# joe5saia/Hmc.jl

Hardware: AMD Instinct MI355X
Metric: Gibbs draws/sec (whole node), 3-state T=1000 x256 windows per GPU (higher is better)
Workload: dtype f64

## Files before the change

### hmc.jl_amd/csrc/gibbs_device.hpp

```cpp
#pragma once
#include <hip/hip_runtime.h>
#include <stdint.h>

#include "../../include/hmcg.h"
#include "round5.hpp"

namespace hmcg {

enum { SITE_SIG2 = 0, SITE_MU = 1, SITE_RHO = 2, SITE_A = 3, SITE_X = 4, SITE_NOISE = 5 };
constexpr int GAMMA_MAX_ATTEMPTS = 64;
constexpr double INVSQRT2PI = 0.3989422804014327;
constexpr double TWO_PI = 6.283185307179586476925286766559;
constexpr double EPS64 = 2.220446049250313e-16;

struct KernelParams {
    const double* Y;
    const int32_t* T;
    const double* yreal;
    int32_t ldY, W, H;
    int32_t sweep_begin;
    int32_t sweep_end;
    int32_t resume;
    int32_t final_launch;
    int32_t horizons[HMCG_MAXH];
    uint32_t seed_lo, seed_hi, window_base;
    double alpha, nu;
    double* mu; double* sig2; double* A; double* pi_end; double* fcast; double* summary;
    int32_t* status;
    const int32_t* x_init; int32_t* x_final; double* pif_final; uint8_t* xstate; double* sumacc;
    const uint32_t* window_ids;
    unsigned long long* dbg;
    int32_t per_sample, burnin_s, nrun_s, n_samples, nd;
    int32_t nd_ld, draw_off;
    double kappa;
    const int32_t* sig_range;
// ... 527 lines not shown

template <int K, int L, int NT, bool SIG>
struct SweepShared {
    static constexpr int NW = NT / 64;
    static constexpr int NCNT = K + K * K;
    static constexpr int NF = K * K + (SIG ? K : 0);
    static constexpr int FW = (64 * L < 1024) ? 10 : 16;
    static constexpr int FPK = 32 / FW;
    static constexpr int NPK = (NF + FPK - 1) / FPK;
    unsigned red_pk[NW][NPK];
    double red_s1[SIG ? NW : 1][K];
    double red_s2[SIG ? NW : 1][K];
    int x_end;
    double red_d1[NW][K];
    double red_d2[NW][K];
    double pivot[K];
    ThetaBuf<K> th[2];
    RngBuf<K> rb[2];
    double wtot[NW][K * K];
    double pfirst[NT + 1][K];
    uint32_t wmap[NW];
    double ulast;
    int xfirst[NT + 1];
    double bred[NW];
    int selcnt[2][8][3];
    double ux[NT * L];
    double exptab[EXPTAB_N * EXPTAB_C];
    struct OutConst { double* base; double yr; int packed; int h; };
    OutConst oc[2][64];
    double ftail[2][SIG ? HMCG_MAXTAIL : 1][K];
    double pf_rep[2][K];
    double y_last[2];
};

template <int NW>
__device__ __forceinline__ double block_sum(double v, double* bred, int wave, int lane)
{
    v = wave_sum(v);
    __syncthreads();
    if (lane == 0 && wave < NW) bred[wave] = v;
    __syncthreads();
    double t = 0.0;
#pragma unroll
    for (int w = 0; w < NW; ++w) t += bred[w];
    return t;
}
template <int NW>
__device__ __forceinline__ double block_minmax(double v, double* bred, int wave, int lane, bool is_max)
{
    v = is_max ? wave_max(v) : wave_min(v);
    __syncthreads();
    if (lane == 0 && wave < NW) bred[wave] = v;
    __syncthreads();
    double t = bred[0];
#pragma unroll
    for (int w = 1; w < NW; ++w) t = is_max ? fmax(t, bred[w]) : fmin(t, bred[w]);
    return t;
}

__device__ __forceinline__ unsigned long long order_key(double v)
{
    const long long b = __double_as_longlong(v + 0.0);
    return (unsigned long long)(b ^ ((b >> 63) | (long long)0x8000000000000000ull));
}
__device__ __forceinline__ double key_value(unsigned long long k)
{
// ... 31 lines not shown
        for (int w = 0; w < NW; ++w) { t0 += cnt[par][w][0]; t1 += cnt[par][w][1]; t2 += cnt[par][w][2]; }
        t0 = __builtin_amdgcn_readfirstlane(t0); t1 = __builtin_amdgcn_readfirstlane(t1); t2 = __builtin_amdgcn_readfirstlane(t2);
        unsigned long long digit = 0ull;
        if (r >= t0) { r -= t0; digit = 1ull;
            if (r >= t1) { r -= t1; digit = 2ull;
                if (r >= t2) { r -= t2; digit = 3ull; } } }
        prefix |= digit << b;
        mask |= 3ull << b;
    }
    return prefix;
}

template <int K>
__device__ __forceinline__ void sort_order(const double (&mu)[K], int (&order)[K])
{
    int pos[K];
#pragma unroll
    for (int i = 0; i < K; ++i) {
        int c = 0;
#pragma unroll
        for (int j = 0; j < K; ++j) c += (mu[j] < mu[i] || (mu[j] == mu[i] && j < i)) ? 1 : 0;
        pos[i] = c;
    }
#pragma unroll
    for (int q = 0; q < K; ++q) {
        int o = 0;
#pragma unroll
        for (int i = 0; i < K; ++i) o += (pos[i] == q) ? i : 0;
        order[q] = o;
    }
}

#ifdef HMCG_STAMPS
#define HMCG_NSTAMP 20
#define HMCG_NSTAMP_ALL (HMCG_NSTAMP + 2)
#define STAMP(i)                                                          \
    do {                                                                  \
        __builtin_amdgcn_sched_barrier(0);                                \
        asm volatile("; HMCG_STAMP_MARK %0" :: "n"(i));                    \
        const unsigned long long t_ = __builtin_amdgcn_s_memtime();       \
        __builtin_amdgcn_s_waitcnt(0xC07F);                               \
        __builtin_amdgcn_sched_barrier(0);                                \
        stamp_acc[i] += t_ - stamp_prev;                                  \
        stamp_prev = t_;                                                  \
    } while (0)
#else
#define STAMP(i)
#endif


template <int K, int L, int NT, bool SIG = false, bool SMOOTH = false, int NH = 0, int OCC = 1>
__global__ __launch_bounds__(NT + 64 * NH) __attribute__((amdgpu_waves_per_eu(OCC)))
void gibbs_sweeps_kernel(const KernelParams p)
{
    static_assert(NH == 0 || (NH == 4 && NT == 256), "helper waves: 256 + 256 threads");
    static_assert(K >= 2 && K <= 4, "small-K kernel: byte-per-entry state maps (v_perm_b32 composition)");
    static_assert(NT % 64 == 0 && NT >= 128, "at least two whole waves (wave 0 draws, the others work in its shadow)");
    constexpr int NW = NT / 64;
    constexpr int KK = K * K;
    constexpr int NG = K + KK;
    static_assert(NG <= 64, "draw roles must fit wave 0");
    using Sh = SweepShared<K, L, NT, SIG>;
    __shared__ Sh sh;

    int w_ = blockIdx.x;
    int t_lo_ = INT32_MIN, t_hi_ = INT32_MAX;
    if (p.order) {
        const int n_live = p.order[0];
        t_lo_ = p.order[1]; t_hi_ = p.order[2];
        if (n_live >= 0) {
            if (w_ >= n_live) __builtin_amdgcn_endpgm();
            w_ = p.order[4 + w_];
        }
    }
    const int w = w_;
    const int tid = threadIdx.x, lane = tid & 63, wave = __builtin_amdgcn_readfirstlane(tid >> 6);
    const int T = p.T[w];
    const int t0 = tid * L;
    const int owner = (T - 1) / L, l_last = (T - 1) % L;
    const bool helper = NH > 0 && __builtin_amdgcn_readfirstlane(wave) >= NW;
    int st = 0;

    if (T < t_lo_ || T > t_hi_) __builtin_amdgcn_endpgm();
    if (T < 2 || T > NT * L || T > p.ldY) {
        if (tid == 0) flag_skipped(p, w, HMCG_ST_BAD_T);
        return;
    }

    exptab_fill(sh.exptab, tid, NT + 64 * NH);
    constexpr int XPAD = K < 4 ? K : 0;
    constexpr bool PADMARK = K < 4;
    double y[L];
    int x[L];
    bool bad = false;
#pragma unroll
// ... 134 lines not shown
            const bool live = task < NTASK;
            const bool t_rho = task < K;
            const bool t_gx = !t_rho && task < K + 2 * NG;
            const bool t_z = !t_rho && !t_gx && task < 2 * K + 2 * NG;
            const bool t_gl = !t_rho && !t_gx && !t_z;
            const int gt = t_gx ? task - K : task - (2 * K + 2 * NG);
            const int role = gt >> 1, j = gt & 1;
            uint32_t site = SITE_RHO, elem = (uint32_t)task, idx = 0;
            if (t_gx || t_gl) {
                site = role < K ? SITE_SIG2 : SITE_A;
                elem = role < K ? (uint32_t)role : (uint32_t)(role - K);
                idx = 2u * (uint32_t)j + (t_gl ? 1u : 0u);
            } else if (t_z) {
                site = SITE_MU; elem = (uint32_t)(task - (K + 2 * NG));
            }
            uint32_t r[4];
            g.block(site, elem, idx, r);
            const double uraw = u53(r[0], r[1]);
            const double lg = log_fast(1.0 - uraw);
            double val = lg;
            if (t_gx || t_z) val = sqrt_fast(-2.0 * lg) * cos2pi_fast(u53(r[2], r[3]));
            double rs = 0.0;
#pragma unroll
            for (int i = 0; i < K; ++i) rs += -__shfl(lg, i, 64);
            if (live) {
                if (t_rho) rb.rho[task] = -lg * (1.0 / rs);
                else if (t_gx) rb.x[role][j] = val;
                else if (t_z) rb.z[task - (K + 2 * NG)] = val;
                else if (t_gl) { rb.lu[role][j] = val; rb.uu[role][j] = uraw; }
            }
        }
    };
    static_assert(NW > 2 || 3 * K + KK <= 64 - 2 * HMCG_MAXH, "parameter and forecast output lanes share a wave when NW == 2");
    auto job_uniforms = [&](int sw, int b0, int b1) __attribute__((always_inline)) {
        Rng g = rng;
        g.sweep = (uint32_t)sw;
        for (int b = b0 + lane; b < b1; b += 128) {
            const int bb = b + 64;
            uint32_t r[4], q[4];
            g.block(SITE_X, 0, (uint32_t)b, r);
            g.block(SITE_X, 0, (uint32_t)bb, q);
            sh.ux[2 * b] = u53(r[0], r[1]);
            if (2 * b + 1 < NT * L) sh.ux[2 * b + 1] = u53(r[2], r[3]);
            if (bb < b1) {
                sh.ux[2 * bb] = u53(q[0], q[1]);
                if (2 * bb + 1 < NT * L) sh.ux[2 * bb + 1] = u53(q[2], q[3]);
            }
        }
    };

    constexpr int FC_SPLIT_MAX = 26;
    double sum_acc = 0.0;
    double smp_acc = 0.0;
    (void)smp_acc;
    constexpr int OUT_WAVE = NH > 0 ? NW + 3 : 1;
    constexpr int FC_WAVE = NH > 0 ? NW + 2 : NW - 1;
    constexpr int PREP_WAVE = NH > 0 ? NW + 1 : (NW - 1 >= 3 ? 2 : 1);
    const int NP = 3 * K + KK;
    auto role_of = [&](int ln) __attribute__((always_inline)) -> int {
        int r = -1;
        if (wave == OUT_WAVE && ln < NP) r = ln;
        if (wave == FC_WAVE && ln >= 64 - 2 * HMCG_MAXH && ln - (64 - 2 * HMCG_MAXH) < 2 * p.H) r = NP + ln - (64 - 2 * HMCG_MAXH);
        return r;
    };
    const int oslot = (wave == FC_WAVE && FC_WAVE != OUT_WAVE) ? 1 : 0;
    if (wave == OUT_WAVE || wave == FC_WAVE) {
        const int orole = role_of(lane);
        double* out_base = nullptr;
        int o_which = 0, o_q = 0, o_i = 0, o_j = 0, fc_h = 0, fc_blend = 0;
        double fc_yr = 0.0;
        const size_t nrun = (size_t)p.nd_ld;
        if (orole >= 0 && orole < 3 * K) {
            o_q = orole % K; o_which = orole / K;
            double* base = o_which == 0 ? p.mu : (o_which == 1 ? p.sig2 : p.pi_end);
            if (base) out_base = base + nrun * ((size_t)o_q + (size_t)K * w);
        } else if (orole >= 3 * K && orole < NP) {
            const int e = orole - 3 * K;
            o_which = 3; o_i = e % K; o_j = e / K;
            if (p.A) out_base = p.A + nrun * ((size_t)e + (size_t)KK * w);
        } else if (orole >= NP) {
// ... 116 lines not shown
                        mine = (c == si) ? g : mine;
                    }
                    val = mine / tot;
                }
            }
        }
        if (out_base) ((__attribute__((address_space(1))) double*)out_base)[d - p.draw_off] = val;
        const double r5 = round5(val);
        sum_acc += r5;
        if constexpr (SIG) {
            if (p.sample_summary) {
                smp_acc += r5;
                const int smp = sw / p.per_sample;
                if (sw + 1 == (smp + 1) * p.per_sample) {
                    const int orole = (c.packed >> 20) & 63;
                    p.sample_summary[((size_t)w * p.n_samples + smp) * NS + orole] = p.nrun_s > 0 ? smp_acc / (double)p.nrun_s : __builtin_nan("");
                    smp_acc = 0.0;
                }
            }
        }
    };

#ifdef HMCG_STAMPS
    unsigned long long stamp_acc[HMCG_NSTAMP];
    unsigned long long stamp_prev = 0;
#endif
    constexpr int PB = L <= 1 ? 1 : (L <= 3 ? 2 : (L <= 7 ? 3 : (L <= 15 ? 4 : 5)));
    constexpr int FPW = 32 / PB;
    constexpr int NF = Sh::NF;
    constexpr int NWORD = (NF + FPW - 1) / FPW;
    constexpr int NPK = Sh::NPK;
    constexpr bool PADCNT = PADMARK && !SIG && NWORD == 1 && NF < FPW;
    static_assert(64 * L < 65536, "wave totals fit their fields (10 bits while 64 L < 1024, else 16)");
    auto publish_stats = [&]() __attribute__((always_inline)) {
        unsigned acc[NWORD];
#pragma unroll
        for (int wd = 0; wd < NWORD; ++wd) acc[wd] = 0;
#pragma unroll
        for (int l = 0; l < L; ++l) {
            const int xn = (l + 1 < L) ? x[(l + 1 < L) ? l + 1 : l] : xnext;
            const int code = PADCNT ? x[l] + K * xn : x[l] * K + xn;
            const bool pv = (t0 + l + 1) < T;
            if constexpr (PADCNT) {
                acc[0] += 1u << (PB * min(code, KK));
            } else if constexpr (NWORD == 1) {
                acc[0] += pv ? (1u << (PB * code)) : 0u;
            } else {
#pragma unroll
                for (int wd = 0; wd < NWORD; ++wd) {
                    const int rel = code - wd * FPW;
                    acc[wd] += (pv && rel >= 0 && rel < FPW) ? (1u << (PB * rel)) : 0u;
                }
            }
            if constexpr (SIG) {
                const int t = t0 + l;
                const bool sv = t >= sb && t < se;
                const int c2 = KK + x[l];
#pragma unroll
                for (int wd = 0; wd < NWORD; ++wd) {
                    const int rel = c2 - wd * FPW;
                    acc[wd] += (sv && rel >= 0 && rel < FPW) ? (1u << (PB * rel)) : 0u;
                }
            }
        }
        unsigned pk[NPK];
#pragma unroll
        for (int d = 0; d < NPK; ++d) {
            unsigned v = 0;
#pragma unroll
            for (int q = 0; q < Sh::FPK; ++q) {
                const int e = Sh::FPK * d + q;
                if (e < NF) v |= ((acc[e / FPW] >> (PB * (e % FPW))) & ((1u << PB) - 1u)) << (Sh::FW * q);
            }
            pk[d] = v;
        }
        wave_sum_words_lane63<NPK>(pk);
        double d1[K], d2[K], s1[SIG ? K : 1], s2[SIG ? K : 1];
#pragma unroll
        for (int i = 0; i < K; ++i) { d1[i] = 0.0; d2[i] = 0.0; }
        if constexpr (SIG) {
#pragma unroll
            for (int i = 0; i < K; ++i) { s1[i] = 0.0; s2[i] = 0.0; }
        }
#pragma unroll
        for (int l = 0; l < L; ++l) {
            double pvt = pivot[0];
#pragma unroll
            for (int k = 1; k < K; ++k) pvt = (x[l] == k) ? pivot[k] : pvt;
            const double dl = y[l] - pvt;
            const int t = t0 + l;
            const bool issig = SIG && t >= sb && t < se;
            const int xs = PADMARK ? (issig ? -1 : x[l]) : ((t < T && !issig) ? x[l] : -1);
#pragma unroll
            for (int i = 0; i < K; ++i) {
                const double dm = (xs == i) ? dl : 0.0;
                d1[i] += dm;
                d2[i] = fma(dm, dm, d2[i]);
            }
            if constexpr (SIG) {
                const int xg = issig ? x[l] : -1;
#pragma unroll
                for (int i = 0; i < K; ++i) {
                    const double dm = (xg == i) ? dl : 0.0;
                    s1[i] += dm;
                    s2[i] = fma(dm, dm, s2[i]);
                }
            }
        }
        if constexpr (SIG) {
// ... 8 lines not shown
                if (i0 < K) dst[i0] = o0;
                if (i1 < K) dst[i1] = o1;
            }
        }
        if constexpr (K <= 4) {
            double v8[8], o0, o1;
#pragma unroll
            for (int i = 0; i < 4; ++i) { v8[i] = i < K ? d1[i] : 0.0; v8[4 + i] = i < K ? d2[i] : 0.0; }
            wave_sum8_transposed(v8, lane, o0, o1);
            if ((lane & 0x3C) == 12) {
                const int i0 = lane & 2, i1 = i0 + 1;
                double* dst = (lane & 1) ? &sh.red_d2[wave][0] : &sh.red_d1[wave][0];
                if (i0 < K) dst[i0] = o0;
                if (i1 < K) dst[i1] = o1;
            }
        } else {
#pragma unroll
            for (int i = 0; i < K; ++i) { d1[i] = wave_sum(d1[i]); d2[i] = wave_sum(d2[i]); }
            if (lane == 0) {
#pragma unroll
                for (int i = 0; i < K; ++i) { sh.red_d1[wave][i] = d1[i]; sh.red_d2[wave][i] = d2[i]; }
            }
        }
        if (lane == 63) {
#pragma unroll
            for (int d = 0; d < NPK; ++d) sh.red_pk[wave][d] = pk[d];
        }
        if (tid == 0) {
#pragma unroll
            for (int k = 0; k < K; ++k) sh.pivot[k] = pivot[k];
            sh.x_end = x_end;
        }
    };
    auto regen_y = [&](int smp, bool report) __attribute__((always_inline)) {
        if constexpr (SIG) {
            const double ssig = p.sigma_signal ? p.sigma_signal[w] : 0.0;
            const bool noisy = ssig != 0.0 || p.n_samples > 1;
            int svb = 0, sve = 0;
            if (p.save_range) { svb = p.save_range[2 * w]; sve = p.save_range[2 * w + 1]; }
            Rng gn = rng;
            gn.sweep = (uint32_t)smp;
#pragma unroll
            for (int l = 0; l < L; ++l) {
                const int t = t0 + l;
                if (noisy && t >= sb && t < se) {
                    uint32_t r[4];
                    gn.block(SITE_NOISE, 0, (uint32_t)t, r);
                    y[l] = yreal[l] + box_muller(r) * ssig;
                }
                if (report && p.sigvals && t >= svb && t < sve && t < T && (t - svb) < p.nsave_ld)
                    p.sigvals[((size_t)w * p.n_samples + smp) * p.nsave_ld + (t - svb)] = y[l];
                if (t == T - 1) sh.y_last[smp & 1] = y[l];
            }
        }
    };
    if constexpr (SIG) {
        if (p.sweep_begin % p.per_sample != 0) regen_y(p.sweep_begin / p.per_sample, false);
    }
    if (!helper) publish_stats();

    if (p.sweep_begin < p.sweep_end && shadow_wave == 0) job_prep(p.sweep_begin);

    uint32_t trips = 0;
    if constexpr (NH > 0) {
        const int ntrip = (((T + 1) >> 1) + 127) >> 7;
        constexpr int trip_wave[10] = {1, 2, 3, NW, 1, 2, 3, NW + 3, NW + 2, NW + 1};
// ... 3 lines not shown
        }
        trips = __builtin_amdgcn_readfirstlane(trips);
    }
    auto job_uniform_trips = [&](int sw) __attribute__((always_inline)) {
        const int nblk = (T + 1) >> 1;
        for (uint32_t m = trips; m != 0; m &= m - 1) {
            const int k = __builtin_ctz(m);
            job_uniforms(sw, k << 7, min((k << 7) + 128, nblk));
        }
    };

    double pf[L][K];
    double sm_acc[SMOOTH ? L : 1][K];
    double fm_acc[SMOOTH ? L : 1][K];
    if constexpr (SMOOTH) {
#pragma unroll
        for (int l = 0; l < L; ++l)
#pragma unroll
            for (int q = 0; q < K; ++q)
            {
                sm_acc[l][q] = (p.resume && p.pi_smooth_mean && t0 + l < T) ? p.pi_smooth_mean[((size_t)w * p.ldY + t0 + l) * K + q] : 0.0;
                fm_acc[l][q] = (p.resume && p.pi_filter_mean && t0 + l < T) ? p.pi_filter_mean[((size_t)w * p.ldY + t0 + l) * K + q] : 0.0;
            }
    }
    (void)sm_acc; (void)fm_acc;
#ifdef HMCG_STAMPS
    for (int i = 0; i < HMCG_NSTAMP; ++i) stamp_acc[i] = 0;
    stamp_prev = __builtin_amdgcn_s_memtime();
    const unsigned long long stamp_t0 = stamp_prev, stamp_r0 = __builtin_amdgcn_s_memrealtime();
#endif

    if constexpr (NH > 0) {
        if (helper) {
            for (int sweep = p.sweep_begin; sweep < p.sweep_end; ++sweep) {
                __syncthreads();
                STAMP(0);
                if (wave == PREP_WAVE && sweep + 1 < p.sweep_end) job_prep(sweep + 1);
                STAMP(15);
                job_uniform_trips(sweep);
                STAMP(1);
                __syncthreads();
                STAMP(2);
                if (sweep > p.sweep_begin) job_outputs(sweep - 1);
                STAMP(14);
                __syncthreads();
                __syncthreads();
                __syncthreads();
                STAMP(11);
            }
        }
    }

    for (int sweep = helper ? p.sweep_end : p.sweep_begin; sweep < p.sweep_end; ++sweep) {
        rng.sweep = (uint32_t)sweep;
        const int par = sweep & 1;
        ThetaBuf<K>& th = sh.th[par];
        if constexpr (SIG) {
            const int smp = sweep / p.per_sample;
            if (sweep == smp * p.per_sample) { regen_y(smp, true); publish_stats(); }
        }
        __syncthreads();
        STAMP(0);
        if (wave == 0) {
            const RngBuf<K>& rb = sh.rb[par];
            const int qi = (lane - 4) >> 2, qj = (lane - 4) & 3;
            const bool is_sig = lane < K, is_A = lane >= 4 && qi < K && qj < K;
            const bool is_g = is_sig || is_A;
            const int role = is_sig ? lane : (is_A ? K + qi * K + qj : NG);
            double shape = 1.0, bpar = 1.0, Neff = 0.0, Ssum = 0.0, rnn = 0.0;
            int cT = 0;
            {
                const int e = is_A ? (PADCNT ? qj * K + qi : role - K) : 0;
#pragma unroll
                for (int ww = 0; ww < NW; ++ww) cT += (int)((sh.red_pk[ww][e / Sh::FPK] >> (Sh::FW * (e % Sh::FPK))) & ((1u << Sh::FW) - 1u));
                cT = is_A ? cT : 0;
            }
            int rowsum = 0;
            {
                int qs = cT + __builtin_amdgcn_mov_dpp(cT, 0xB1, 0xF, 0xF, false);
                qs += __builtin_amdgcn_mov_dpp(qs, 0x4E, 0xF, 0xF, false);
#pragma unroll
                for (int i = 0; i < K; ++i) {
                    const int ri = __builtin_amdgcn_readlane(qs, 4 + 4 * i);
                    rowsum = (lane == i) ? ri : rowsum;
                }
            }
            STAMP(16);
            if (is_g) {
                const int c = is_sig ? rowsum + ((sh.x_end == role) ? 1 : 0) : cT;
                if (is_sig) {
                    double d1 = 0.0, d2 = 0.0;
#pragma unroll
                    for (int ww = 0; ww < NW; ++ww) { d1 += sh.red_d1[ww][role]; d2 += sh.red_d2[ww][role]; }
                    const double piv = sh.pivot[role];
                    const double beta = (sweep == 0) ? 1.0 : 2.0;
                    if constexpr (!SIG) {
                        Neff = (double)c;
                        const double rn = c > 0 ? rcp_fast(Neff) : 0.0;
                        const double ybar = c > 0 ? piv + d1 * rn : 0.0;
                        const double S2 = c > 0 ? fmax(d2 - d1 * d1 * rn, 0.0) : 0.0;
                        Ssum = piv * Neff + d1;
                        const double dm = ybar - xi;
                        shape = p.alpha + 0.5 * Neff;
                        rnn = rcp_fast(Neff + p.nu);
                        bpar = beta + 0.5 * S2 + 0.5 * Neff * p.nu * rnn * (dm * dm);
                    } else {
                        int Mi = 0;
                        {
                            const int e = KK + role;
#pragma unroll
                            for (int ww = 0; ww < NW; ++ww) Mi += (int)((sh.red_pk[ww][e / Sh::FPK] >> (Sh::FW * (e % Sh::FPK))) & ((1u << Sh::FW) - 1u));
                        }
                        const int Ni = c - Mi;
                        double g1 = 0.0, g2 = 0.0;
#pragma unroll
                        for (int ww = 0; ww < NW; ++ww) { g1 += sh.red_s1[ww][role]; g2 += sh.red_s2[ww][role]; }
                        const double dNi = (double)Ni, dMi = (double)Mi;
                        const double S = piv * dNi + d1, Sm = piv * dMi + g1;
                        const double S2 = Ni > 0 ? fmax(d2 - d1 * d1 / dNi, 0.0) : 0.0;
                        const double Sm2 = Mi > 0 ? fmax(g2 - g1 * g1 / dMi, 0.0) : 0.0;
                        const double totalbar = (Ni + Mi) > 0 ? (S + Sm) / (dNi + dMi) : 0.0;
                        Neff = dNi + dMi * kfac;
                        Ssum = S + Sm;
                        const double dm = totalbar - xi;
                        shape = p.alpha + 0.5 * dNi + 0.5 * dMi;
                        rnn = rcp_fast(Neff + p.nu);
                        bpar = beta + 0.5 * S2 + (0.5 * kfac) * Sm2 + 0.5 * Neff * p.nu * rnn * (dm * dm);
                    }
                } else {
                    shape = (double)(c + 1);
                }
            }
            STAMP(17);
            double val = 1.0;
            if (is_g) {
                const uint32_t site = role < K ? SITE_SIG2 : SITE_A;
                const uint32_t elem = role < K ? (uint32_t)role : (uint32_t)(role - K);
                if (shape == 1.0) {
                    uint32_t r[4];
                    rng.block(site, elem, 0, r);
                    val = -log_fast(1.0 - u53(r[0], r[1]));
                } else {
                    const double a = shape < 1.0 ? shape + 1.0 : shape;
                    const double dd = a - 1.0 / 3.0;
                    const double cc = rsqrt_fast(dd) * (1.0 / 3.0);
                    val = mt_try(dd, cc, rb.x[role][0], rb.lu[role][0], rb.uu[role][0]);
                    if (val < 0.0) val = mt_try(dd, cc, rb.x[role][1], rb.lu[role][1], rb.uu[role][1]);
                    if (val < 0.0) {
                        int j = 2;
                        for (; j < GAMMA_MAX_ATTEMPTS && val < 0.0; ++j) {
                            uint32_t r[4];
                            rng.block(site, elem, 2u * (uint32_t)j, r);
                            const double xx = box_muller(r);
                            rng.block(site, elem, 2u * (uint32_t)j + 1u, r);
                            const double u3 = u53(r[0], r[1]);
                            val = mt_try(dd, cc, xx, log_fast(1.0 - u3), u3);
                        }
                        if (val < 0.0) { val = dd; st |= HMCG_ST_GAMMA_CAP; }
                    }
                    if (shape < 1.0) {
                        uint32_t r[4];
                        rng.block(site, elem, 0xFFFFFFFFu, r);
                        val *= pow(1.0 - u53(r[0], r[1]), 1.0 / shape);
                    }
                }
            }
            STAMP(18);
            double gs = is_A ? val : 0.0;
            gs += quadperm_f64<0xB1>(gs);
            gs += quadperm_f64<0x4E>(gs);
            if (is_sig) {
                const double sig2 = bpar * rcp_fast(val);
                const double m = (Ssum + p.nu * xi) * rnn;
                const double sdev = sqrt_fast(sig2 * rnn);
                const double mu = m + sdev * rb.z[role];
                const double isd = rsqrt_fast(sig2);
                th.mu[role] = mu; th.sig2[role] = sig2;
                th.isd[role] = isd * 0.70710678118654752440; th.coef[role] = INVSQRT2PI * isd;
                th.rho[role] = rb.rho[role];
            } else if (is_A) {
                th.A[qi][qj] = val * rcp_fast(gs);
            }
        } else {
            const int nblk = (T + 1) >> 1;
            if (sweep > p.sweep_begin) job_outputs(sweep - 1);
            STAMP(14);
            if constexpr (NH > 0) {
                job_uniform_trips(sweep);
            } else if (NSH >= 3) {
                const int extra = NSH - 3;
                const int c_last = (nblk * 3) / 16;
                const int rest = nblk - c_last;
                const int den = 2 * (8 + 5) + 13 * extra;
                const int c0 = (rest * 16) / den, c1 = (rest * 10) / den;
                int b0, b1;
                if (shadow_wave == 0) { b0 = 0; b1 = c0; }
                else if (shadow_wave == 1) { b0 = c0; b1 = extra > 0 ? c0 + c1 : rest; }
                else if (shadow_wave == NSH - 1) { b0 = rest; b1 = nblk; }
                else {
                    const int per = extra > 0 ? (rest - c0 - c1 + extra - 1) / extra : 0;
                    b0 = c0 + c1 + (shadow_wave - 2) * per;
                    b1 = min(b0 + per, rest);
                }
                if (shadow_wave == 1 && sweep + 1 < p.sweep_end) job_prep(sweep + 1);
                STAMP(15);
                job_uniforms(sweep, b0, b1);
            } else {
                if (shadow_wave == 0 && sweep + 1 < p.sweep_end) job_prep(sweep + 1);
                const int per = (nblk + NSH - 1) / NSH;
                job_uniforms(sweep, shadow_wave * per, min((shadow_wave + 1) * per, nblk));
            }
        }
        STAMP(1);
        __syncthreads();
        STAMP(2);
        double mu[K], isd[K], coef[K], rho[K], A[K][K];
        int order[K];
#pragma unroll
        for (int i = 0; i < K; ++i) {
            mu[i] = th.mu[i]; isd[i] = th.isd[i]; coef[i] = th.coef[i]; rho[i] = th.rho[i];
#pragma unroll
            for (int j = 0; j < K; ++j) A[i][j] = th.A[i][j];
        }
        sort_order<K>(mu, order);
        double ux[L];
#pragma unroll
        for (int l = 0; l < L; ++l) ux[l] = sh.ux[t0 + l];
        double f[L][K];
        unsigned und = 0;
        if constexpr (L >= 8) {
#pragma unroll
            for (int l = 0; l < L; ++l) {
                unsigned hm = 0;
#pragma unroll
                for (int s = 0; s < K; ++s) {
                    double z = (y[l] - mu[s]) * isd[s];
                    double cf = coef[s];
                    if constexpr (SIG) {
                        const bool issig = (t0 + l) >= sb && (t0 + l) < se;
                        z = issig ? z * kfac : z;
                        cf = issig ? cf * kfac : cf;
                    }
                    f[l][s] = exp_tab(-(z * z), sh.exptab, lane & (EXPTAB_C - 1)) * cf;
                    hm = max(hm, (unsigned)__double2hiint(f[l][s]));
                }
                const int e = 1022 - (int)(hm >> 20);
#pragma unroll
                for (int s = 0; s < K; ++s) f[l][s] = ldexp(f[l][s], e);
                und |= (hm < 0x01A56E1Fu) ? (1u << l) : 0u;
            }
        } else {
            constexpr int LB = (16 / K) < L ? (16 / K) : L;
#define HMCG_EACH for (int g = 0; g < LB; ++g) _Pragma("unroll") for (int s = 0; s < K; ++s)
#define HMCG_SB __builtin_amdgcn_sched_barrier(0)
#pragma unroll
            for (int l0 = 0; l0 < L; l0 += LB) {
                double x[LB][K], nn[LB][K], tj[LB][K], r[LB][K], pp[LB][K];
                int ni[LB][K];
                auto LL = [&](int g) __attribute__((always_inline)) { return l0 + g < L ? l0 + g : L - 1; };
                auto issig = [&](int g) __attribute__((always_inline)) { return SIG && (t0 + LL(g)) >= sb && (t0 + LL(g)) < se; };
// ... 376 lines not shown
        Hm = bmap_compose(Hm, (uint32_t)dpp_i32<DPP_ROW_SHL1, 0xF>((int)BMAP_IDENTITY, (int)Hm));
        Hm = bmap_compose(Hm, (uint32_t)dpp_i32<DPP_ROW_SHL2, 0xF>((int)BMAP_IDENTITY, (int)Hm));
        Hm = bmap_compose(Hm, (uint32_t)dpp_i32<DPP_ROW_SHL4, 0xF>((int)BMAP_IDENTITY, (int)Hm));
        Hm = bmap_compose(Hm, (uint32_t)dpp_i32<DPP_ROW_SHL8, 0xF>((int)BMAP_IDENTITY, (int)Hm));
        {
            const uint32_t R1 = (uint32_t)__builtin_amdgcn_readlane((int)Hm, 16);
            const uint32_t R2 = (uint32_t)__builtin_amdgcn_readlane((int)Hm, 32);
            const uint32_t R3 = (uint32_t)__builtin_amdgcn_readlane((int)Hm, 48);
            const uint32_t S1 = bmap_compose(R2, R3), S0 = bmap_compose(R1, S1);
            const int row = lane >> 4;
            const uint32_t after = row == 0 ? S0 : (row == 1 ? S1 : (row == 2 ? R3 : BMAP_IDENTITY));
            Hm = bmap_compose(Hm, after);
        }
        if (lane == 0) sh.wmap[wave] = Hm;
        STAMP(10);
        __syncthreads();
        STAMP(11);
        uint32_t Rw = BMAP_IDENTITY;
#pragma unroll
        for (int ww = NW - 1; ww >= 1; --ww) if (ww > wave_u) Rw = bmap_compose(sh.wmap[ww], Rw);
        const uint32_t Hx = (uint32_t)dpp_i32<DPP_WAVE_SHL1, 0xF>((int)BMAP_IDENTITY, (int)Hm);
        const uint32_t Sfx = bmap_compose(Hx, Rw);
        int sin = bmap_apply(Sfx, XPAD);
        xnext = sin;
        x_end = xlast;
#pragma unroll
        for (int l = L - 1; l >= 0; --l) {
            sin = bmap_apply(gmap[l], sin);
            x[l] = sin;
        }
#pragma unroll
        for (int k = 0; k < K; ++k) pivot[k] = mu[k];
        STAMP(12);
        publish_stats();
        STAMP(13);
    }
#ifdef HMCG_STAMPS
    if (lane == 0 && p.dbg) {
        unsigned long long* o = p.dbg + ((size_t)w * (NW + NH) + wave) * HMCG_NSTAMP_ALL;
        for (int i = 0; i < HMCG_NSTAMP; ++i) o[i] = stamp_acc[i];
        o[HMCG_NSTAMP] = __builtin_amdgcn_s_memtime() - stamp_t0;
        o[HMCG_NSTAMP + 1] = __builtin_amdgcn_s_memrealtime() - stamp_r0;
    }
#endif

    __syncthreads();
    if (p.sweep_end > p.sweep_begin) job_outputs(p.sweep_end - 1);
    if (p.xstate) {
#pragma unroll
        for (int l = 0; l < L; ++l) if (t0 + l < T) p.xstate[(size_t)w * p.ldY + t0 + l] = (uint8_t)x[l];
    }
    if (p.x_final) {
#pragma unroll
        for (int l = 0; l < L; ++l) if (t0 + l < T) p.x_final[(size_t)w * p.ldY + t0 + l] = x[l];
    }
    if (p.pif_final && p.sweep_end > p.sweep_begin) {
#pragma unroll
        for (int l = 0; l < L; ++l)
            if (t0 + l < T)
#pragma unroll
                for (int s = 0; s < K; ++s) p.pif_final[((size_t)w * p.ldY + t0 + l) * K + s] = pf[l][s];
    }
    if constexpr (SMOOTH) {
        if (p.pi_filter_mean) {
            const double sc = (p.final_launch && p.nd > 0) ? 1.0 / (double)p.nd : 1.0;
#pragma unroll
            for (int l = 0; l < L; ++l)
                if (t0 + l < T)
// ... 35 lines not shown
```

### hmc.jl_amd/csrc/hmcg.hip

```cpp
#include <hip/hip_runtime.h>

#include <algorithm>
#include <chrono>
#include <cstdarg>
#include <cstdlib>
#include <cstdio>
#include <cstring>
#include <functional>
#include <mutex>
#include <string>
#include <thread>
#include <vector>

#include "gibbs_device.hpp"
#include "host_util.hpp"
#include "moments.hpp"
#include "plan.hpp"

namespace {

thread_local char g_err[512] = "";

void set_err(const char* fmt, ...)
{
// ... 299 lines not shown
            HIP_TRY(hipGetLastError());
            if (b > 0) HIP_TRY(hipEventRecord(c.ev_join[b - 1], bs));
        }
        for (int b = 1; b < pl.nb; ++b) HIP_TRY(hipStreamWaitEvent(stream, c.ev_join[b - 1], 0));
        return 0;
    }
    if (pl.v) hipLaunchKernelGGL(pl.v->fn, dim3((unsigned)p.W), dim3((unsigned)(pl.v->NT + 64 * pl.v->NH)), 0, stream, p);
    else hipLaunchKernelGGL(pl.bv->fn, dim3((unsigned)p.W), dim3((unsigned)pl.bv->NT), pl.dyn, stream, p, pl.bigL);
    HIP_TRY(hipGetLastError());
    return 0;
}

void fill_timing(hmcg_timing* t, const Plan& pl, const DeviceCtx& c, double kernel_ms, int launches, double call_ms, int windows)
{
    if (!t) return;
    t->kernel_ms = kernel_ms;
    t->launches = launches;
    t->threads_per_window = pl.NT();
    t->steps_per_thread = pl.L();
    t->helper_waves = pl.NH();
    t->device = c.device;
    t->call_ms = call_ms;
    t->windows = windows;
    t->occupancy = pl.v ? pl.v->occ : 0;
    t->buckets = pl.nb > 1 ? pl.nb : 1;
    t->streaming = pl.stream ? 1 : 0;
    t->lds_bytes = (int32_t)(static_lds_bytes(pl.fptr(), 0) + pl.dyn);
}

#ifdef HMCG_STAMPS
int print_stamps(const hmcg::KernelParams& p, const Plan& pl, unsigned long long* ddbg, size_t ndbg, hipStream_t stream)
{
    static const char* names[HMCG_NSTAMP] = {"Ba wait", "param draws | shadow jobs", "Bb wait", "theta+ux+pdfs", "local product",
        "wave scan", "Bc wait", "prefix+replay+last", "Bd wait", "maps+compose", "map scan", "Be wait", "apply", "publish stats", "  (shadow: outputs)", "  (shadow: prep)", "  (param: counts+row sums)", "  (param: shapes)", "  (param: gamma)", "unused"};
    const int nwv = pl.NT() / 64 + pl.NH();
    std::vector<unsigned long long> h(ndbg);
    HIP_TRY(hipStreamSynchronize(stream));
    static int launches_seen = 0;
    static const int print_after = diag_env("HMCG_STAMPS_AFTER") ? atoi(diag_env("HMCG_STAMPS_AFTER")) : 0;
    if (launches_seen++ < print_after) return 0;
    HIP_TRY(hipMemcpy(h.data(), ddbg, ndbg * sizeof(unsigned long long), hipMemcpyDeviceToHost));
    const int nsw = p.sweep_end - p.sweep_begin;
    {
        std::vector<double> clk;
        double ticks = 0;
        for (int w = 0; w < p.W; ++w)
            for (int wv = 0; wv < nwv; ++wv) {
                const unsigned long long* o = &h[((size_t)w * nwv + wv) * HMCG_NSTAMP_ALL];
                if (o[HMCG_NSTAMP + 1]) { clk.push_back(100.0 * (double)o[HMCG_NSTAMP] / (double)o[HMCG_NSTAMP + 1]); ticks += (double)o[HMCG_NSTAMP]; }
            }
        std::sort(clk.begin(), clk.end());
        if (!clk.empty())
            fprintf(stderr, "[clock] launch %d: in-kernel clock MHz min %.0f median %.0f max %.0f (s_memtime / s_memrealtime x 100 MHz); "
                            "%.0f ticks per sweep (mean over waves)\n", launches_seen - 1, clk.front(), clk[clk.size() / 2], clk.back(),
                    ticks / (double)clk.size() / (nsw > 0 ? nsw : 1));
    }
    fprintf(stderr, "[stamps] K=%d L=%d NT=%d W=%d sweeps=%d: mean cycles per sweep by wave (s_memtime ticks)\n",
            pl.v ? pl.v->K : pl.bv->K, pl.L(), pl.NT(), p.W, nsw);
    fprintf(stderr, "%-24s", "phase");
    for (int wv = 0; wv < nwv; ++wv) fprintf(stderr, "   wave%-2d", wv);
    fprintf(stderr, "\n");
    std::vector<double> tot(nwv, 0.0);
    for (int i = 0; i < HMCG_NSTAMP; ++i) {
        fprintf(stderr, "%-24s", names[i]);
        for (int wv = 0; wv < nwv; ++wv) {
            double acc = 0;
            for (int w = 0; w < p.W; ++w) acc += (double)h[((size_t)w * nwv + wv) * HMCG_NSTAMP_ALL + i];
// ... 504 lines not shown
```

Baseline: 54.49 million.

## Split publish stats into counts and sums and double-buffer uniforms across sweeps

For helper-wave kernels with L==4, the end-of-sweep statistics publish is split. Transition counts are published immediately, while the residual sums are deferred to the next sweep, where a helper wave computes wave 0's share from packed states. The uniform draws are double-buffered in shared memory so helpers can generate part of the next sweep's uniforms ahead of time. Parameter draws now span an extra barrier so the gamma draw overlaps the deferred sum reduction. This shortens the critical path at the cost of more LDS, an extra barrier per sweep and more complex cross-sweep ordering.

Result: faster. 56.41 million, median of 6 (+3.5%).

```diff
diff --git a/hmc.jl_amd/csrc/gibbs_device.hpp b/hmc.jl_amd/csrc/gibbs_device.hpp
--- a/hmc.jl_amd/csrc/gibbs_device.hpp
+++ b/hmc.jl_amd/csrc/gibbs_device.hpp
@@ -1,6 +1,7 @@
 #pragma once
 #include <hip/hip_runtime.h>
 #include <stdint.h>
+#include <type_traits>
 
 #include "../../include/hmcg.h"
 #include "round5.hpp"
@@ -594,6 +595,11 @@
     double pf_rep[2][K];
     double y_last[2];
 };
+template <int K, int L, int NT>
+struct SweepSharedSplit : SweepShared<K, L, NT, false> {
+    unsigned xw0[64];
+    double ux2[NT * L];
+};
 
 template <int NW>
 __device__ __forceinline__ double block_sum(double v, double* bred, int wave, int lane)
@@ -691,7 +697,7 @@
 }
 
 #ifdef HMCG_STAMPS
-#define HMCG_NSTAMP 20
+#define HMCG_NSTAMP 23
 #define HMCG_NSTAMP_ALL (HMCG_NSTAMP + 2)
 #define STAMP(i)                                                          \
     do {                                                                  \
@@ -719,7 +725,9 @@
     constexpr int KK = K * K;
     constexpr int NG = K + KK;
     static_assert(NG <= 64, "draw roles must fit wave 0");
-    using Sh = SweepShared<K, L, NT, SIG>;
+    constexpr bool SPLIT = NH > 0 && !SIG && L == 4;
+    static_assert(!SPLIT || (NH == 4 && NT * L <= 1024), "SPLIT deals exactly four uniform trips: three to helpers NW+1..NW+3, one ahead");
+    using Sh = typename std::conditional<SPLIT, SweepSharedSplit<K, L, NT>, SweepShared<K, L, NT, SIG>>::type;
     __shared__ Sh sh;
 
     int w_ = blockIdx.x;
@@ -920,20 +928,37 @@
         }
     };
     static_assert(NW > 2 || 3 * K + KK <= 64 - 2 * HMCG_MAXH, "parameter and forecast output lanes share a wave when NW == 2");
+    auto ux_of = [&](int sw) __attribute__((always_inline)) -> double* {
+        if constexpr (SPLIT) return (sw & 1) ? sh.ux2 : sh.ux;
+        else return sh.ux;
+    };
     auto job_uniforms = [&](int sw, int b0, int b1) __attribute__((always_inline)) {
         Rng g = rng;
         g.sweep = (uint32_t)sw;
+        double* const ub = ux_of(sw);
         for (int b = b0 + lane; b < b1; b += 128) {
             const int bb = b + 64;
             uint32_t r[4], q[4];
             g.block(SITE_X, 0, (uint32_t)b, r);
             g.block(SITE_X, 0, (uint32_t)bb, q);
-            sh.ux[2 * b] = u53(r[0], r[1]);
-            if (2 * b + 1 < NT * L) sh.ux[2 * b + 1] = u53(r[2], r[3]);
+            ub[2 * b] = u53(r[0], r[1]);
+            if (2 * b + 1 < NT * L) ub[2 * b + 1] = u53(r[2], r[3]);
             if (bb < b1) {
-                sh.ux[2 * bb] = u53(q[0], q[1]);
-                if (2 * bb + 1 < NT * L) sh.ux[2 * bb + 1] = u53(q[2], q[3]);
-            }
+                ub[2 * bb] = u53(q[0], q[1]);
+                if (2 * bb + 1 < NT * L) ub[2 * bb + 1] = u53(q[2], q[3]);
+            }
+        }
+    };
+    auto job_uniforms_half = [&](int sw, int b0, int b1) __attribute__((always_inline)) {
+        Rng g = rng;
+        g.sweep = (uint32_t)sw;
+        double* const ub = ux_of(sw);
+        const int b = b0 + lane;
+        if (b < b1) {
+            uint32_t r[4];
+            g.block(SITE_X, 0, (uint32_t)b, r);
+            ub[2 * b] = u53(r[0], r[1]);
+            if (2 * b + 1 < NT * L) ub[2 * b + 1] = u53(r[2], r[3]);
         }
     };
 
@@ -1116,7 +1141,11 @@
     constexpr int NPK = Sh::NPK;
     constexpr bool PADCNT = PADMARK && !SIG && NWORD == 1 && NF < FPW;
     static_assert(64 * L < 65536, "wave totals fit their fields (10 bits while 64 L < 1024, else 16)");
-    auto publish_stats = [&]() __attribute__((always_inline)) {
+    auto publish = [&](auto with_counts, auto with_sums, const int (&xs_)[L], const double (&pv)[K], int tq0, int dw) __attribute__((always_inline)) {
+        constexpr bool COUNTS = decltype(with_counts)::value, SUMS = decltype(with_sums)::value;
+        static_assert(COUNTS != SUMS, "one half at a time: publish_stats is the whole");
+        unsigned pk[NPK];
+        if constexpr (COUNTS) {
         unsigned acc[NWORD];
 #pragma unroll
         for (int wd = 0; wd < NWORD; ++wd) acc[wd] = 0;
@@ -1147,7 +1176,6 @@
                 }
             }
         }
-        unsigned pk[NPK];
 #pragma unroll
         for (int d = 0; d < NPK; ++d) {
             unsigned v = 0;
@@ -1159,6 +1187,131 @@
             pk[d] = v;
         }
         wave_sum_words_lane63<NPK>(pk);
+        }
+        if constexpr (SUMS) {
+        double d1[K], d2[K], s1[SIG ? K : 1], s2[SIG ? K : 1];
+#pragma unroll
+        for (int i = 0; i < K; ++i) { d1[i] = 0.0; d2[i] = 0.0; }
+        if constexpr (SIG) {
+#pragma unroll
+            for (int i = 0; i < K; ++i) { s1[i] = 0.0; s2[i] = 0.0; }
+        }
+#pragma unroll
+        for (int l = 0; l < L; ++l) {
+            double pvt = pv[0];
+#pragma unroll
+            for (int k = 1; k < K; ++k) pvt = (xs_[l] == k) ? pv[k] : pvt;
+            const double dl = y[l] - pvt;
+            const int t = tq0 + l;
+            const bool issig = SIG && t >= sb && t < se;
+            const int xs = PADMARK ? (issig ? -1 : xs_[l]) : ((t < T && !issig) ? xs_[l] : -1);
+#pragma unroll
+            for (int i = 0; i < K; ++i) {
+                const double dm = (xs == i) ? dl : 0.0;
+                d1[i] += dm;
+                d2[i] = fma(dm, dm, d2[i]);
+            }
+            if constexpr (SIG) {
+                const int xg = issig ? xs_[l] : -1;
+#pragma unroll
+                for (int i = 0; i < K; ++i) {
+                    const double dm = (xg == i) ? dl : 0.0;
+                    s1[i] += dm;
+                    s2[i] = fma(dm, dm, s2[i]);
+                }
+            }
+        }
+        if constexpr (SIG) {
+            static_assert(!SIG || K <= 4, "signal path: transposed reduce carries 2 x 4 slots");
+            double v8[8], o0, o1;
+#pragma unroll
+            for (int i = 0; i < 4; ++i) { v8[i] = i < K ? s1[i < K ? i : 0] : 0.0; v8[4 + i] = i < K ? s2[i < K ? i : 0] : 0.0; }
+            wave_sum8_transposed(v8, lane, o0, o1);
+            if ((lane & 0x3C) == 12) {
+                const int i0 = lane & 2, i1 = i0 + 1;
+                double* dst = (lane & 1) ? &sh.red_s2[dw][0] : &sh.red_s1[dw][0];
+                if (i0 < K) dst[i0] = o0;
+                if (i1 < K) dst[i1] = o1;
+            }
+        }
+        if constexpr (K <= 4) {
+            double v8[8], o0, o1;
+#pragma unroll
+            for (int i = 0; i < 4; ++i) { v8[i] = i < K ? d1[i] : 0.0; v8[4 + i] = i < K ? d2[i] : 0.0; }
+            wave_sum8_transposed(v8, lane, o0, o1);
+            if ((lane & 0x3C) == 12) {
+                const int i0 = lane & 2, i1 = i0 + 1;
+                double* dst = (lane & 1) ? &sh.red_d2[dw][0] : &sh.red_d1[dw][0];
+                if (i0 < K) dst[i0] = o0;
+                if (i1 < K) dst[i1] = o1;
+            }
+        } else {
+#pragma unroll
+            for (int i = 0; i < K; ++i) { d1[i] = wave_sum(d1[i]); d2[i] = wave_sum(d2[i]); }
+            if (lane == 0) {
+#pragma unroll
+                for (int i = 0; i < K; ++i) { sh.red_d1[dw][i] = d1[i]; sh.red_d2[dw][i] = d2[i]; }
+            }
+        }
+        }
+        if constexpr (COUNTS) {
+            if (lane == 63) {
+#pragma unroll
+                for (int d = 0; d < NPK; ++d) sh.red_pk[wave][d] = pk[d];
+            }
+        }
+        if (COUNTS ? tid == 0 : (dw == 0 && lane == 0)) {
+            if constexpr (SUMS) {
+#pragma unroll
+                for (int k = 0; k < K; ++k) sh.pivot[k] = pv[k];
+            }
+            if constexpr (COUNTS) sh.x_end = x_end;
+        }
+    };
+    auto publish_stats = [&]() __attribute__((always_inline)) {
+        unsigned acc[NWORD];
+#pragma unroll
+        for (int wd = 0; wd < NWORD; ++wd) acc[wd] = 0;
+#pragma unroll
+        for (int l = 0; l < L; ++l) {
+            const int xn = (l + 1 < L) ? x[(l + 1 < L) ? l + 1 : l] : xnext;
+            const int code = PADCNT ? x[l] + K * xn : x[l] * K + xn;
+            const bool pv = (t0 + l + 1) < T;
+            if constexpr (PADCNT) {
+                acc[0] += 1u << (PB * min(code, KK));
+            } else if constexpr (NWORD == 1) {
+                acc[0] += pv ? (1u << (PB * code)) : 0u;
+            } else {
+#pragma unroll
+                for (int wd = 0; wd < NWORD; ++wd) {
+                    const int rel = code - wd * FPW;
+                    acc[wd] += (pv && rel >= 0 && rel < FPW) ? (1u << (PB * rel)) : 0u;
+                }
+            }
+            if constexpr (SIG) {
+                const int t = t0 + l;
+                const bool sv = t >= sb && t < se;
+                const int c2 = KK + x[l];
+#pragma unroll
+                for (int wd = 0; wd < NWORD; ++wd) {
+                    const int rel = c2 - wd * FPW;
+                    acc[wd] += (sv && rel >= 0 && rel < FPW) ? (1u << (PB * rel)) : 0u;
+                }
+            }
+        }
+        unsigned pk[NPK];
+#pragma unroll
+        for (int d = 0; d < NPK; ++d) {
+            unsigned v = 0;
+#pragma unroll
+            for (int q = 0; q < Sh::FPK; ++q) {
+                const int e = Sh::FPK * d + q;
+                if (e < NF) v |= ((acc[e / FPW] >> (PB * (e % FPW))) & ((1u << PB) - 1u)) << (Sh::FW * q);
+            }
+            pk[d] = v;
+        }
+        wave_sum_words_lane63<NPK>(pk);
+        STAMP(19);
         double d1[K], d2[K], s1[SIG ? K : 1], s2[SIG ? K : 1];
 #pragma unroll
         for (int i = 0; i < K; ++i) { d1[i] = 0.0; d2[i] = 0.0; }
@@ -1233,6 +1386,11 @@
             sh.x_end = x_end;
         }
     };
+    auto publish_counts = [&]() __attribute__((always_inline)) { publish(std::true_type(), std::false_type(), x, pivot, t0, wave); };
+    auto publish_sums = [&](const int (&xs_)[L], const double (&pv)[K], int tq0, int dw) __attribute__((always_inline)) {
+        publish(std::false_type(), std::true_type(), xs_, pv, tq0, dw);
+    };
+    (void)publish_counts; (void)publish_sums;
     auto regen_y = [&](int smp, bool report) __attribute__((always_inline)) {
         if constexpr (SIG) {
             const double ssig = p.sigma_signal ? p.sigma_signal[w] : 0.0;
@@ -1302,15 +1460,53 @@
 
     if constexpr (NH > 0) {
         if (helper) {
+            if constexpr (SPLIT) {
+                if (wave == NW) {
+#pragma unroll
+                    for (int l = 0; l < L; ++l) y[l] = (lane * L + l) < T ? p.Y[(size_t)w * p.ldY + lane * L + l] : 0.0;
+                }
+            }
             for (int sweep = p.sweep_begin; sweep < p.sweep_end; ++sweep) {
                 __syncthreads();
                 STAMP(0);
-                if (wave == PREP_WAVE && sweep + 1 < p.sweep_end) job_prep(sweep + 1);
-                STAMP(15);
-                job_uniform_trips(sweep);
-                STAMP(1);
-                __syncthreads();
-                STAMP(2);
+                if constexpr (SPLIT) {
+                    const bool first = sweep == p.sweep_begin;
+                    const int nblk = (T + 1) >> 1;
+                    const int hb = (wave - (NW + 1)) * 128;
+                    if (wave == NW && !first) {
+                        const unsigned xw = sh.xw0[lane];
+                        int hx[L];
+                        double hp[K];
+#pragma unroll
+                        for (int l = 0; l < L; ++l) hx[l] = (int)((xw >> (2 * l)) & 3u);
+#pragma unroll
+                        for (int k = 0; k < K; ++k) hp[k] = sh.th[(sweep & 1) ^ 1].mu[k];
+                        publish_sums(hx, hp, lane * L, 0);
+                    }
+                    STAMP(13);
+                    if (first) job_uniform_trips(sweep);
+                    else if (hb >= 0) job_uniforms_half(sweep, hb, min(hb + 64, nblk));
+                    STAMP(1);
+                    __syncthreads();
+                    STAMP(20);
+                    if (!first && hb >= 0) job_uniforms_half(sweep, hb + 64, min(hb + 128, nblk));
+                    STAMP(21);
+                    __syncthreads();
+                    STAMP(2);
+                    if (sweep + 1 < p.sweep_end) {
+                        if (wave == PREP_WAVE) job_prep(sweep + 1);
+                        STAMP(15);
+                        if (wave == NW) job_uniforms(sweep + 1, 3 * 128, min(4 * 128, nblk));
+                        STAMP(22);
+                    }
+                } else {
+                    if (wave == PREP_WAVE && sweep + 1 < p.sweep_end) job_prep(sweep + 1);
+                    STAMP(15);
+                    job_uniform_trips(sweep);
+                    STAMP(1);
+                    __syncthreads();
+                    STAMP(2);
+                }
                 if (sweep > p.sweep_begin) job_outputs(sweep - 1);
                 STAMP(14);
                 __syncthreads();
@@ -1359,6 +1555,11 @@
             if (is_g) {
                 const int c = is_sig ? rowsum + ((sh.x_end == role) ? 1 : 0) : cT;
                 if (is_sig) {
+                    if constexpr (SPLIT) {
+                        Neff = (double)c;
+                        shape = p.alpha + 0.5 * Neff;
+                        rnn = rcp_fast(Neff + p.nu);
+                    } else {
                     double d1 = 0.0, d2 = 0.0;
 #pragma unroll
                     for (int ww = 0; ww < NW; ++ww) { d1 += sh.red_d1[ww][role]; d2 += sh.red_d2[ww][role]; }
@@ -1396,6 +1597,7 @@
                         shape = p.alpha + 0.5 * dNi + 0.5 * dMi;
                         rnn = rcp_fast(Neff + p.nu);
                         bpar = beta + 0.5 * S2 + (0.5 * kfac) * Sm2 + 0.5 * Neff * p.nu * rnn * (dm * dm);
+                    }
                     }
                 } else {
                     shape = (double)(c + 1);
@@ -1439,8 +1641,29 @@
             double gs = is_A ? val : 0.0;
             gs += quadperm_f64<0xB1>(gs);
             gs += quadperm_f64<0x4E>(gs);
+            if constexpr (SPLIT) {
+                if (is_sig) val = rcp_fast(val);
+                if (is_A) th.A[qi][qj] = val * rcp_fast(gs);
+                STAMP(1);
+                __syncthreads();
+                STAMP(20);
+                if (is_sig) {
+                    const int c = rowsum + ((sh.x_end == role) ? 1 : 0);
+                    double d1 = 0.0, d2 = 0.0;
+#pragma unroll
+                    for (int ww = 0; ww < NW; ++ww) { d1 += sh.red_d1[ww][role]; d2 += sh.red_d2[ww][role]; }
+                    const double piv = sh.pivot[role];
+                    const double beta = (sweep == 0) ? 1.0 : 2.0;
+                    const double rn = c > 0 ? rcp_fast(Neff) : 0.0;
+                    const double ybar = c > 0 ? piv + d1 * rn : 0.0;
+                    const double S2 = c > 0 ? fmax(d2 - d1 * d1 * rn, 0.0) : 0.0;
+                    Ssum = piv * Neff + d1;
+                    const double dm = ybar - xi;
+                    bpar = beta + 0.5 * S2 + 0.5 * Neff * p.nu * rnn * (dm * dm);
+                }
+            }
             if (is_sig) {
-                const double sig2 = bpar * rcp_fast(val);
+                const double sig2 = bpar * (SPLIT ? val : rcp_fast(val));
                 const double m = (Ssum + p.nu * xi) * rnn;
                 const double sdev = sqrt_fast(sig2 * rnn);
                 const double mu = m + sdev * rb.z[role];
@@ -1448,14 +1671,23 @@
                 th.mu[role] = mu; th.sig2[role] = sig2;
                 th.isd[role] = isd * 0.70710678118654752440; th.coef[role] = INVSQRT2PI * isd;
                 th.rho[role] = rb.rho[role];
-            } else if (is_A) {
+            } else if (!SPLIT && is_A) {
                 th.A[qi][qj] = val * rcp_fast(gs);
             }
         } else {
             const int nblk = (T + 1) >> 1;
+            if constexpr (SPLIT) {
+                if (sweep > p.sweep_begin) publish_sums(x, pivot, t0, wave);
+                STAMP(13);
+            }
             if (sweep > p.sweep_begin) job_outputs(sweep - 1);
             STAMP(14);
-            if constexpr (NH > 0) {
+            if constexpr (SPLIT) {
+                if (sweep == p.sweep_begin) job_uniform_trips(sweep);
+                STAMP(1);
+                __syncthreads();
+                STAMP(20);
+            } else if constexpr (NH > 0) {
                 job_uniform_trips(sweep);
             } else if (NSH >= 3) {
                 const int extra = NSH - 3;
@@ -1481,7 +1713,7 @@
                 job_uniforms(sweep, shadow_wave * per, min((shadow_wave + 1) * per, nblk));
             }
         }
-        STAMP(1);
+        if constexpr (SPLIT) { STAMP(21); } else { STAMP(1); }
         __syncthreads();
         STAMP(2);
         double mu[K], isd[K], coef[K], rho[K], A[K][K];
@@ -1495,7 +1727,7 @@
         sort_order<K>(mu, order);
         double ux[L];
 #pragma unroll
-        for (int l = 0; l < L; ++l) ux[l] = sh.ux[t0 + l];
+        for (int l = 0; l < L; ++l) ux[l] = ux_of(sweep)[t0 + l];
         double f[L][K];
         unsigned und = 0;
         if constexpr (L >= 8) {
@@ -1938,8 +2170,19 @@
 #pragma unroll
         for (int k = 0; k < K; ++k) pivot[k] = mu[k];
         STAMP(12);
-        publish_stats();
-        STAMP(13);
+        if constexpr (SPLIT) {
+            publish_counts();
+            if (wave == 0) {
+                unsigned xw = 0;
+#pragma unroll
+                for (int l = 0; l < L; ++l) xw |= (unsigned)x[l] << (2 * l);
+                sh.xw0[lane] = xw;
+            }
+            STAMP(19);
+        } else {
+            publish_stats();
+            STAMP(13);
+        }
     }
 #ifdef HMCG_STAMPS
     if (lane == 0 && p.dbg) {
diff --git a/hmc.jl_amd/csrc/hmcg.hip b/hmc.jl_amd/csrc/hmcg.hip
--- a/hmc.jl_amd/csrc/hmcg.hip
+++ b/hmc.jl_amd/csrc/hmcg.hip
@@ -355,7 +355,7 @@
 int print_stamps(const hmcg::KernelParams& p, const Plan& pl, unsigned long long* ddbg, size_t ndbg, hipStream_t stream)
 {
     static const char* names[HMCG_NSTAMP] = {"Ba wait", "param draws | shadow jobs", "Bb wait", "theta+ux+pdfs", "local product",
-        "wave scan", "Bc wait", "prefix+replay+last", "Bd wait", "maps+compose", "map scan", "Be wait", "apply", "publish stats", "  (shadow: outputs)", "  (shadow: prep)", "  (param: counts+row sums)", "  (param: shapes)", "  (param: gamma)", "unused"};
+        "wave scan", "Bc wait", "prefix+replay+last", "Bd wait", "maps+compose", "map scan", "Be wait", "apply", "publish sums", "  (shadow: outputs)", "  (shadow: prep)", "  (param: counts+row sums)", "  (param: shapes)", "  (param: gamma)", "  (stats: counts)", "Ba2 wait", "param finish | half trips", "  (shadow: ux ahead)"};
     const int nwv = pl.NT() / 64 + pl.NH();
     std::vector<unsigned long long> h(ndbg);
     HIP_TRY(hipStreamSynchronize(stream));
```
